# simplify23/MRN

Hardware: NVIDIA B200
Metric: MRN-SVTR 6-expert train samples/s (higher is better)
Workload: dtype bf16

## Files before the change

mrn_b200/csrc/mixer_tc.cu:

```cuda
#include "mixer_tc.h"
#include "sm100.cuh"
#include <stdlib.h>
#include <type_traits>

namespace {

#ifndef MRNB_MIXER_OVL
#define MRNB_MIXER_OVL 1
#endif
constexpr int HD = 32;
constexpr int EPI_WARPS = 8, NTHREADS = 512;
constexpr int REGS_CTRL = 80, REGS_SOFTMAX = 168, REGS_EPI = 96;
constexpr uint32_t Y_COL = 0, S0_COL = 256, S1_COL = 320, O0_COL = 384, O1_COL = 416, STG0_COL = 256, STG1_COL = 352;
constexpr uint32_t STGX_COL = 448;

__device__ __forceinline__ void pair_sync(int q) {
  switch (q) {
    case 0: asm volatile("bar.sync 1, 64;" ::: "memory"); break;
    case 1: asm volatile("bar.sync 2, 64;" ::: "memory"); break;
    case 2: asm volatile("bar.sync 3, 64;" ::: "memory"); break;
    default: asm volatile("bar.sync 4, 64;" ::: "memory"); break;
  }
}
template <int D>
struct MCfg {
  static constexpr int N = 32768 / D;
  static constexpr int NT = N / 128;
  static constexpr int KR = N / 64;
  static constexpr int HEADS = D / HD;
  static constexpr int KB = D / 64;
  static constexpr int A_BYTES = ((D == 128 && MRNB_MIXER_OVL) ? 128 : N) * D * 2;
  static constexpr int HT_BYTES = 128 * HD * 2;
  static constexpr bool OVL = D == 128 && MRNB_MIXER_OVL;
  static constexpr int QKV1_BYTES = 3 * NT * HT_BYTES;
  static constexpr int QKV_BYTES = (OVL ? 2 : 1) * QKV1_BYTES;
  static constexpr int P_TILE = 128 * 64 * 2;
  static constexpr int P_BYTES = 2 * P_TILE;
  static constexpr int WQ_KB_BYTES = 96 * 128;
  static constexpr int WQ_BYTES = KB * WQ_KB_BYTES;
  static constexpr int WP_BYTES = D * HD * 2;
  static constexpr int STG_BYTES = 4 * 2048;
  static constexpr int BIAS_BYTES = OVL ? 4 * 3 * D * 4 : 0;
  static constexpr int SMEM = 1024 + A_BYTES + QKV_BYTES + P_BYTES + WQ_BYTES + 2 * WP_BYTES + STG_BYTES + BIAS_BYTES;
  static_assert(NT * D == 256, "Y accumulator spans 256 TMEM columns");
  static_assert(SMEM <= 227 * 1024, "shared memory budget");
};

struct MixParams {
  const float* bqkv; const float* bproj;
  float* x; long x_gs;
  const float* rowscale; long rs_gs;
  __nv_bfloat16* ln_out; const float* ln_gamma; const float* ln_beta; float ln_eps;
  int upg, total;
  int dbg;
  unsigned long long* trace;
};

#define MIX_TRACE(slot_, idx_)                                                                     \
  do {                                                                                             \
    if (ep.trace && blockIdx.x == 0 && (idx_) < 256) {                                             \
      unsigned long long now__;                                                                    \
      asm volatile("mov.u64 %0, %%globaltimer;" : "=l"(now__));                                    \
      ep.trace[(slot_) * 256 + (idx_)] = now__;                                                    \
    }                                                                                              \
  } while (0)

template <int D, bool LNF, int LNU = 2>
__device__ __forceinline__ void y_tile_epilogue(const MixParams& ep, int e, long unit, int qt, int q, int lane, uint32_t y_addr,
                                                float* xt, float rs, float* stg, uint64_t* release) {
  const int rsub = lane >> 2, c4 = lane & 3;
  const float* bpj = ep.bproj + (long)e * D;
  float sum[4] = {0.f, 0.f, 0.f, 0.f}, sq[4] = {0.f, 0.f, 0.f, 0.f};
  float4 xin[4], xnx[4];
  if (!(ep.dbg & 2)) {
#pragma unroll
// ... 139 lines not shown
      }
    }
    __syncwarp();
  }
}

template <int D, bool LOCAL, bool LNF>
__global__ void __launch_bounds__(NTHREADS, 1)
mixer_tc_kernel(const __grid_constant__ CUtensorMap tmA, const __grid_constant__ CUtensorMap tmWq,
                const __grid_constant__ CUtensorMap tmWp, const MixParams ep) {
  using K = MCfg<D>;
  extern __shared__ uint8_t smem_raw[];
  uint8_t* smem = smem_raw + align_smem_1024_offset(smem_raw);
  uint8_t* sA = smem;
  uint8_t* sQ = sA + K::A_BYTES;
  uint8_t* sK = sQ + K::NT * K::HT_BYTES;
  uint8_t* sV = sK + K::NT * K::HT_BYTES;
  uint8_t* sP = sQ + K::QKV_BYTES;
  uint8_t* sWq = sP + K::P_BYTES;
  uint8_t* sWp = sWq + K::WQ_BYTES;
  uint8_t* sStg = sWp + 2 * K::WP_BYTES;
  float* sBias = reinterpret_cast<float*>(sStg + K::STG_BYTES);
  __shared__ __align__(8) uint64_t a_full, a_empty, wq_full, wq_empty, wp_full[2], wp_empty[2], stg_full[2], stg_empty[2], qkv_ready,
      s_full[2], s_empty[2], p_full[2], o_full[2], so_full[2], so_empty[2], y_full, y_empty[4], st1_done, qkvr[2], qkvf[2], yd[2];
  __shared__ uint32_t tmem_base_sh;
  __shared__ float ln_part[2][4][2][32];

  const int warp = threadIdx.x >> 5, lane = threadIdx.x & 31;
  const int total = ep.total, upg = ep.upg;

  if (threadIdx.x == 0) {
    mbar_init(&a_full, 1); mbar_init(&a_empty, 1); mbar_init(&wq_full, 1); mbar_init(&wq_empty, 1);
    for (int b = 0; b < 2; ++b) {
      mbar_init(&wp_full[b], 1); mbar_init(&wp_empty[b], 2);
      mbar_init(&stg_full[b], 1); mbar_init(&stg_empty[b], K::OVL ? 4 : EPI_WARPS);
      mbar_init(&qkvr[b], 128); mbar_init(&qkvf[b], 2); mbar_init(&yd[b], 1);
      mbar_init(&s_full[b], 1); mbar_init(&s_empty[b], 128); mbar_init(&p_full[b], 128); mbar_init(&o_full[b], 1);
      mbar_init(&so_full[b], 128); mbar_init(&so_empty[b], 1);
    }
    mbar_init(&qkv_ready, EPI_WARPS * 32); mbar_init(&y_full, 2); mbar_init(&st1_done, 1);
    for (int b = 0; b < 4; ++b) mbar_init(&y_empty[b], 4);
    fence_mbarrier_init();
    prefetch_tmap(&tmA);
    prefetch_tmap(&tmWq);
    prefetch_tmap(&tmWp);
  }
  if (warp == 1) tmem_alloc(&tmem_base_sh, 512);
  tc_fence_before();
  __syncthreads();
  tc_fence_after();
  const uint32_t tmem_base = tmem_base_sh;

  auto kr_lo = [](int qt) { return LOCAL ? (2 * qt - 3 > 0 ? 2 * qt - 3 : 0) : 0; };
  auto kr_hi = [](int qt) { return LOCAL ? (2 * qt + 5 < K::KR ? 2 * qt + 5 : K::KR) : K::KR; };

  if (warp < 4) asm volatile("setmaxnreg.dec.sync.aligned.u32 %0;" ::"n"(REGS_CTRL));
  if (warp == 0) {
    if (lane == 0) {
      if constexpr (K::OVL) {
        uint32_t hc = 0, tc = 0;
        for (int u = blockIdx.x; u < total; u += gridDim.x) {
          const int e = u / upg;
          for (int h = 0; h < K::HEADS; ++h, ++hc) {
            mbar_wait(&wq_empty, (hc & 1u) ^ 1u);
            mbar_expect_tx(&wq_full, K::WQ_BYTES);
            for (int kb = 0; kb < K::KB; ++kb)
              for (int part = 0; part < 3; ++part)
                tma_load_3d(sWq + kb * K::WQ_KB_BYTES + part * 4096, &tmWq, &wq_full, kb * 64, part * D + h * HD, e);
            const int buf = hc & 1u;
            mbar_wait(&wp_empty[buf], ((hc >> 1) & 1u) ^ 1u);
            mbar_expect_tx(&wp_full[buf], K::WP_BYTES);
            tma_load_3d(sWp + buf * K::WP_BYTES, &tmWp, &wp_full[buf], h * HD, 0, e);
            for (int mt = 0; mt < K::NT; ++mt, ++tc) {
              mbar_wait(&a_empty, (tc & 1u) ^ 1u);
              mbar_expect_tx(&a_full, K::A_BYTES);
              for (int kb = 0; kb < K::KB; ++kb) tma_load_3d(sA + kb * 16384, &tmA, &a_full, kb * 64, mt * 128, u);
            }
          }
        }
      } else {
      uint32_t hc = 0;
      int i = 0;
      for (int u = blockIdx.x; u < total; u += gridDim.x, ++i) {
        const int e = u / upg;
        mbar_wait(&a_empty, ((uint32_t)i & 1u) ^ 1u);
        mbar_expect_tx(&a_full, K::A_BYTES);
        for (int mt = 0; mt < K::NT; ++mt)
          for (int kb = 0; kb < K::KB; ++kb) tma_load_3d(sA + (mt * K::KB + kb) * 16384, &tmA, &a_full, kb * 64, mt * 128, u);
        for (int h = 0; h < K::HEADS; ++h, ++hc) {
          mbar_wait(&wq_empty, (hc & 1u) ^ 1u);
          mbar_expect_tx(&wq_full, K::WQ_BYTES);
          for (int kb = 0; kb < K::KB; ++kb)
            for (int part = 0; part < 3; ++part)
              tma_load_3d(sWq + kb * K::WQ_KB_BYTES + part * 4096, &tmWq, &wq_full, kb * 64, part * D + h * HD, e);
          const int buf = hc & 1u;
          mbar_wait(&wp_empty[buf], ((hc >> 1) & 1u) ^ 1u);
          mbar_expect_tx(&wp_full[buf], K::WP_BYTES);
          tma_load_3d(sWp + buf * K::WP_BYTES, &tmWp, &wp_full[buf], h * HD, 0, e);
        }
      }
      }
    }
  } else if (warp == 3) {
    if constexpr (K::OVL) {
      if (lane == 0) {
        constexpr uint32_t idesc_qk = umma_idesc(UMMA_BF16, 128, 64), idesc_v = umma_idesc(UMMA_BF16, 128, 32);
        uint32_t hc = 0, tc = 0, pc = 0;
        for (int u = blockIdx.x; u < total; u += gridDim.x) {
          for (int h = 0; h < K::HEADS; ++h, ++hc) {
            mbar_wait(&wq_full, hc & 1u);
            tc_fence_after();
            for (int mt = 0; mt < K::NT; ++mt, ++tc) {
              mbar_wait(&a_full, tc & 1u);
              tc_fence_after();
#pragma unroll
              for (int part = 0; part < 2; ++part, ++pc) {
                mbar_wait(&stg_empty[0], (pc & 1u) ^ 1u);
                tc_fence_after();
                for (int kb = 0; kb < K::KB; ++kb) {
                  const uint64_t ad = umma_desc_k128(smem_u32(sA + kb * 16384));
                  const uint64_t bd = umma_desc_k128(smem_u32(sWq + kb * K::WQ_KB_BYTES + part * 8192));
#pragma unroll
                  for (int k = 0; k < 4; ++k)
                    umma_bf16(tmem_base + STGX_COL, ad + (uint64_t)(k * 2), bd + (uint64_t)(k * 2), part ? idesc_v : idesc_qk, (kb | k) != 0);
                }
                umma_commit(&stg_full[0]);
              }
              umma_commit(&a_empty);
            }
            umma_commit(&wq_empty);
          }
        }
      }
    }
  } else if (warp == 1 || warp == 2) {
    if (lane == 0) {
      const int s = warp == 1 ? 0 : 1;
      constexpr uint32_t idesc_qkv = umma_idesc(UMMA_BF16, 128, 96), idesc_s = umma_idesc(UMMA_BF16, 128, 64);
      constexpr uint32_t idesc_o = umma_idesc(UMMA_BF16, 128, HD, false, true), idesc_y = umma_idesc(UMMA_BF16, 128, D);
      const uint32_t s_col = s ? S1_COL : S0_COL, o_col = s ? O1_COL : O0_COL;
      uint32_t hc = 0, mc = 0, pc = 0, qc = 0;
      bool s_early = false;
      int i = 0;
      for (int u = blockIdx.x; u < total; u += gridDim.x, ++i) {
        if (!K::OVL && s == 0) { mbar_wait(&a_full, (uint32_t)i & 1u); tc_fence_after(); }
        for (int h = 0; h < K::HEADS; ++h, ++hc) {
          if (!K::OVL && s == 0) {
            mbar_wait(&wq_full, hc & 1u);
            mbar_wait(&st1_done, (hc & 1u) ^ 1u);
            tc_fence_after();
            for (int mt = 0; mt < K::NT; ++mt, ++mc) {
              const uint32_t sb = mc & 1u, stg_col = sb ? STG1_COL : STG0_COL;
              mbar_wait(&stg_empty[sb], ((mc >> 1) & 1u) ^ 1u);
              tc_fence_after();
              for (int kb = 0; kb < K::KB; ++kb) {
                const uint64_t ad = umma_desc_k128(smem_u32(sA + (mt * K::KB + kb) * 16384));
                const uint64_t bd = umma_desc_k128(smem_u32(sWq + kb * K::WQ_KB_BYTES));
#pragma unroll
                for (int k = 0; k < 4; ++k) umma_bf16(tmem_base + stg_col, ad + (uint64_t)(k * 2), bd + (uint64_t)(k * 2), idesc_qkv, (kb | k) != 0);
              }
              umma_commit(&stg_full[sb]);
            }
            umma_commit(&wq_empty);
            if (h == K::HEADS - 1) umma_commit(&a_empty);
          }
          const int buf = hc & 1u;
          if constexpr (K::OVL) { if (!s_early) mbar_wait(&qkvr[buf], (hc >> 1) & 1u); }
          else mbar_wait(&qkv_ready, hc & 1u);
// ... 42 lines not shown
                const bool more = !(h == K::HEADS - 1 && u + (int)gridDim.x >= total);
                const uint32_t nb = (hc + 1u) & 1u;
                if (!has_next && more && mbar_test(&qkvr[nb], ((hc + 1u) >> 1) & 1u)) {
                  mbar_wait(&s_empty[s], (pc - 1u) & 1u);
                  tc_fence_after();
                  issue_s_from(sQ + nb * K::QKV1_BYTES, sK + nb * K::QKV1_BYTES, s, kr_lo(s));
                  s_early = true;
                }
              }
              if (last_of_tile) {
                mbar_wait(&so_full[s], qc & 1u);
                tc_fence_after();
                if (!K::OVL && h == 0) { mbar_wait(&y_empty[qt], ((uint32_t)i & 1u) ^ 1u); tc_fence_after(); }
                const uint64_t od = umma_smem_desc(smem_u32(sP + s * K::P_TILE), 16, 512, UMMA_SWIZZLE_64B);
                const uint64_t wd = umma_smem_desc(smem_u32(sWp + buf * K::WP_BYTES), 16, 512, UMMA_SWIZZLE_64B);
#pragma unroll
                for (int k = 0; k < HD / 16; ++k)
                  umma_bf16(tmem_base + Y_COL + (uint32_t)(qt * D), od + (uint64_t)(k * 2), wd + (uint64_t)(k * 2), idesc_y, (h | k) != 0);
                umma_commit(&so_empty[s]);
                if (K::OVL && h == K::HEADS - 1) umma_commit(&yd[s]);
                ++qc;
              }
              if (!has_next) break;
              qt = nqt; kr = nkr;
            }
          }
          umma_commit(&wp_empty[buf]);
          if (s == 1) umma_commit(&st1_done);
          if constexpr (K::OVL) umma_commit(&qkvf[buf]);
        }
        if (!K::OVL) umma_commit(&y_full);
      }
    }
  } else if (warp >= 4 && warp < 12) {
    asm volatile("setmaxnreg.inc.sync.aligned.u32 %0;" ::"n"(REGS_SOFTMAX));
    const int ew = warp - 4, q = warp & 3, ch = ew >> 2;
    const int r = q * 32 + lane;
    const uint32_t lane_addr = tmem_base + ((uint32_t)(q * 32) << 16);
    const int sw = (r >> 1) & 3;
    const float sl2 = 0.17677669529663688110f * 1.4426950408889634f;
    uint8_t* ptile = sP + ch * K::P_TILE;
    float* stg = reinterpret_cast<float*>(ptile + (size_t)q * 4096);
    const int p8 = lane & 7, rsel = lane >> 3;
    constexpr int OW = D / 2, NPASS = OW / 32;
    const uint32_t s_col = ch ? S1_COL : S0_COL, o_col = ch ? O1_COL : O0_COL;
    uint32_t hc = 0, mc = 0, pc = 0, qc = 0;
    int i = 0;
    for (int u = blockIdx.x; u < total; u += gridDim.x, ++i) {
      const int e = u / upg, b = u % upg;
      if constexpr (K::OVL) {
        const char* xl2 = reinterpret_cast<const char*>(ep.x + (long)e * ep.x_gs + (long)b * K::N * D + (long)(ch * 128) * D);
#pragma unroll
        for (int k = 0; k < D / 32; ++k) asm volatile("prefetch.global.L2 [%0];" ::"l"(xl2 + (long)(k * 128 + q * 32 + lane) * 128));
      }
      for (int h = 0; h < K::HEADS; ++h, ++hc) {
        if constexpr (!K::OVL) {
        float bias[3][16];
#pragma unroll
        for (int pi = 0; pi < 3; ++pi) {
          const int p = ch * 3 + pi;
          const float4* bp = reinterpret_cast<const float4*>(ep.bqkv + (long)e * 3 * D + (p >> 1) * D + h * HD + (p & 1) * 16);
#pragma unroll
          for (int j = 0; j < 4; ++j) {
            const float4 t = __ldg(bp + j);
            bias[pi][4 * j] = t.x; bias[pi][4 * j + 1] = t.y; bias[pi][4 * j + 2] = t.z; bias[pi][4 * j + 3] = t.w;
          }
        }
// ... 136 lines not shown
          }
          const float inv = 1.0f / l;
          {
            uint8_t* row = ptile + r * 64;
#pragma unroll
            for (int c4 = 0; c4 < 4; ++c4) {
              uint32_t pk[4];
#pragma unroll
              for (int k2 = 0; k2 < 4; ++k2) pk[k2] = pack_bf16(acc[c4 * 8 + 2 * k2] * inv, acc[c4 * 8 + 2 * k2 + 1] * inv);
              *reinterpret_cast<uint4*>(row + ((c4 ^ sw) * 16)) = make_uint4(pk[0], pk[1], pk[2], pk[3]);
            }
          }
          asm volatile("fence.proxy.async.shared::cta;" ::: "memory");
          mbar_arrive(&so_full[ch]);
          if constexpr (K::OVL) {
            if (h == K::HEADS - 1) {
              if (warp == 4 && lane == 0) MIX_TRACE(11, i);
              const float rs = ep.rowscale ? ep.rowscale[(long)e * ep.rs_gs + b] : 1.0f;
              float* xt = ep.x + (long)e * ep.x_gs + (long)b * K::N * D + (long)(qt * 128 + q * 32) * D;
              if (ep.dbg == 0) {
                y_tile_epilogue_regs<D, LNF, 2>(ep, e, u, qt, q, lane, lane_addr + Y_COL + (uint32_t)(qt * D), xt, rs, stg, 0, 2, &yd[ch], (uint32_t)i & 1u, nullptr);
              } else {
                mbar_wait(&yd[ch], (uint32_t)i & 1u);
                tc_fence_after();
                y_tile_epilogue<D, LNF, 8>(ep, e, u, qt, q, lane, lane_addr + Y_COL + (uint32_t)(qt * D), xt, rs, stg, nullptr);
              }
              tc_fence_before();
              if (warp == 4 && lane == 0) MIX_TRACE(13, i);
            }
          }
        }
      }

    }
  } else if (warp >= 12) {
    asm volatile("setmaxnreg.dec.sync.aligned.u32 %0;" ::"n"(REGS_EPI));
    const int q = warp & 3;
    const uint32_t lane_addr = tmem_base + ((uint32_t)(q * 32) << 16);
    float* stg = reinterpret_cast<float*>(sStg + q * 2048);
    const int rsub = lane >> 2, c4 = lane & 3;
    int d_u = blockIdx.x, d_h = 0, d_part = 0, d_e = -1;
    uint32_t d_pc = 0, d_hc = 0;
    float* wbias = sBias + q * 3 * D;
    auto try_drain = [&]() -> bool {
      if constexpr (!K::OVL) return false;
      if (d_u >= total) return false;
      mbar_wait(&stg_full[0], d_pc & 1u);
      const int hb = d_hc & 1u;
      if (d_part == 0) {
        mbar_wait(&qkvf[hb], ((d_hc >> 1) & 1u) ^ 1u);
        const int e = d_u / upg;
        if (e != d_e) {
          __syncwarp();
          for (int k = lane; k < 3 * D; k += 32) wbias[k] = ep.bqkv[(long)e * 3 * D + k];
          __syncwarp();
          d_e = e;
        }
      }
      tc_fence_after();
      const int mt = d_part >> 1, part = d_part & 1;
      const int r = q * 32 + lane, sw = (r >> 1) & 3;
      uint8_t* qkv = sQ + hb * K::QKV1_BYTES;
      const int nt = part ? 1 : 2;
      for (int tt = 0; tt < nt; ++tt) {
        uint32_t v[32];
        tmem_ld32(lane_addr + STGX_COL + (uint32_t)(tt * 32), v);
        if (tt == nt - 1) {
          tc_fence_before();
          __syncwarp();
          if (lane == 0) mbar_arrive(&stg_empty[0]);
        }
        const int t = part ? 2 : tt;
        const float4* bp = reinterpret_cast<const float4*>(wbias + t * D + d_h * HD);
        uint8_t* row = qkv + (size_t)t * K::NT * K::HT_BYTES + mt * K::HT_BYTES + r * 64;
#pragma unroll
        for (int c = 0; c < 4; ++c) {
          const float4 b0 = bp[2 * c], b1 = bp[2 * c + 1];
          *reinterpret_cast<uint4*>(row + ((c ^ sw) * 16)) = make_uint4(
              pack_bf16(__uint_as_float(v[8 * c]) + b0.x, __uint_as_float(v[8 * c + 1]) + b0.y),
              pack_bf16(__uint_as_float(v[8 * c + 2]) + b0.z, __uint_as_float(v[8 * c + 3]) + b0.w),
              pack_bf16(__uint_as_float(v[8 * c + 4]) + b1.x, __uint_as_float(v[8 * c + 5]) + b1.y),
              pack_bf16(__uint_as_float(v[8 * c + 6]) + b1.z, __uint_as_float(v[8 * c + 7]) + b1.w));
        }
      }
      ++d_pc;
      if (++d_part == 2 * K::NT) {
        asm volatile("fence.proxy.async.shared::cta;" ::: "memory");
        mbar_arrive(&qkvr[hb]);
        if (warp == 12 && lane == 0) MIX_TRACE(14, (int)d_hc);
        d_part = 0; ++d_hc;
        if (++d_h == K::HEADS) { d_h = 0; d_u += gridDim.x; }
      }
      return true;
    };
    if constexpr (K::OVL) {
      while (d_u < total) try_drain();
    } else {
    int i = 0;
    for (int u = blockIdx.x; u < total; u += gridDim.x, ++i) {
      const int e = u / upg, b = u % upg;
      const float rs = ep.rowscale ? ep.rowscale[(long)e * ep.rs_gs + b] : 1.0f;
      float* xunit = ep.x + (long)e * ep.x_gs + (long)b * K::N * D;
      {
        const char* xl2 = reinterpret_cast<const char*>(xunit);
#pragma unroll
        for (int k = 0; k < 8; ++k) asm volatile("prefetch.global.L2 [%0];" ::"l"(xl2 + ((long)(k * 128 + (threadIdx.x - 384))) * 128));
      }
      mbar_wait(&y_full, (uint32_t)i & 1u);
      tc_fence_after();
      if (warp == 12 && lane == 0) MIX_TRACE(11, i);
// ... 30 lines not shown
  using K = MCfg<D>;
  const long units = (long)p.groups * p.units_per_group;
  CUtensorMap tmA, tmWq, tmWp;
  MRNB_TRY(map3(&tmA, p.A, D, K::N, units, 64, 128, CU_TENSOR_MAP_SWIZZLE_128B));
  MRNB_TRY(map3(&tmWq, p.Wqkv, D, 3 * D, p.groups, 64, 32, CU_TENSOR_MAP_SWIZZLE_128B));
  MRNB_TRY(map3(&tmWp, p.Wproj, D, D, p.groups, 32, D, CU_TENSOR_MAP_SWIZZLE_64B));
  MixParams ep{};
  ep.bqkv = p.bqkv; ep.bproj = p.bproj; ep.x = p.x; ep.x_gs = p.x_gstride;
  ep.rowscale = p.rowscale; ep.rs_gs = p.rowscale_gstride;
  ep.ln_out = (__nv_bfloat16*)p.ln_out; ep.ln_gamma = p.ln_gamma; ep.ln_beta = p.ln_beta; ep.ln_eps = p.ln_eps;
  ep.upg = p.units_per_group; ep.total = (int)units;
  { const char* e = getenv("MRNB_MIXER_DBG"); ep.dbg = e ? atoi(e) : 0; }
  ep.trace = (unsigned long long*)g_mixer_trace;
  static bool attr = false;
  static int num_sms = 148;
  if (!attr) {
    cudaFuncSetAttribute(mixer_tc_kernel<D, LOCAL, LNF>, cudaFuncAttributeMaxDynamicSharedMemorySize, K::SMEM);
    int dev = 0;
    cudaGetDevice(&dev);
    cudaDeviceGetAttribute(&num_sms, cudaDevAttrMultiProcessorCount, dev);
    attr = true;
  }
  const int grid = units < num_sms ? (int)units : num_sms;
  mixer_tc_kernel<D, LOCAL, LNF><<<grid, NTHREADS, K::SMEM, st>>>(tmA, tmWq, tmWp, ep);
  MRNB_CHECK_LAUNCH("mixer_tc_kernel");
  return MRNB_OK;
}

}

int mrnb_mixer_tc(const MrnbMixer& p, cudaStream_t st) {
  MRNB_CHECK_ARG(p.A && p.Wqkv && p.bqkv && p.Wproj && p.bproj && p.x && p.groups > 0 && p.units_per_group > 0, "mixer_tc: null/empty argument");
  MRNB_CHECK_ARG(p.D == 64 || p.D == 128 || p.D == 256, "mixer_tc: D must be 64, 128 or 256");
  MRNB_CHECK_ARG(!p.ln_out || (p.D <= 128 && p.ln_gamma && p.ln_beta), "mixer_tc: fused LayerNorm needs D <= 128");
  MRNB_CHECK_ARG(!(p.local && p.D == 256), "mixer_tc: the Local mixer exists for the 64- and 128-wide stages only");
  MRNB_CHECK_ARG(p.x_gstride % 4 == 0, "mixer_tc: misaligned residual stream");
  const double units = (double)p.groups * p.units_per_group, N = 32768.0 / p.D;
  MrnbProfScope prof(MRNB_PROF_MIXER, st, units * (8.0 * N * p.D * p.D + 4.0 * N * N * p.D),
                     units * N * p.D * (2.0 + 8.0 + (p.ln_out ? 2.0 : 0.0)));
#define MRNB_MIX(D_, LOC_) return p.ln_out ? launch_mixer<D_, LOC_, true>(p, st) : launch_mixer<D_, LOC_, false>(p, st);
  if (p.D == 64) { if (p.local) { MRNB_MIX(64, true) } MRNB_MIX(64, false) }
  if (p.D == 128) { if (p.local) { MRNB_MIX(128, true) } MRNB_MIX(128, false) }
  return launch_mixer<256, false, false>(p, st);
#undef MRNB_MIX
}

extern "C" void mrnb_mixer_set_trace(void* device_buffer) { g_mixer_trace = device_buffer; }

extern "C" int mrnb_mixer_bf16(const void* A, const void* Wqkv, const float* bqkv, const void* Wproj, const float* bproj,
                               float* x, const float* rowscale, void* ln_out, const float* ln_gamma, const float* ln_beta,
                               float ln_eps, int units, int D, int local, cudaStream_t stream) {
  MrnbMixer p{};
  p.A = A; p.Wqkv = Wqkv; p.bqkv = bqkv; p.Wproj = Wproj; p.bproj = bproj; p.x = x; p.x_gstride = 0;
  p.rowscale = rowscale; p.rowscale_gstride = 0;
  p.ln_out = ln_out; p.ln_gamma = ln_gamma; p.ln_beta = ln_beta; p.ln_eps = ln_eps;
  p.D = D; p.groups = 1; p.units_per_group = units; p.local = local;
  return mrnb_mixer_tc(p, stream);
}
```

mrn_b200/csrc/svtr.cu:

```cuda
#include "common.cuh"
#include "gemm_f32.h"
#include "gemm_tc.h"
#include "mlp_tc.h"
#include "mixer_tc.h"
#include <stdlib.h>
#include "svtr.h"
#include "expert_util.cuh"

int mrnb_attention_tc(const void* qkv, void* out, int groups, int N, int d, int heads, int H, int W, int local, cudaStream_t st);

namespace {

template <typename OT, int D, int RPW = 4>
__global__ void __launch_bounds__(256)
layernorm_kernel(const float* x, long x_gs, OT* y, long y_gs, const float* __restrict__ gamma,
                 const float* __restrict__ beta, long rows, long rows_per_group, float eps,
                 __nv_bfloat16* __restrict__ y2 = nullptr, long y2_gs = 0, const float* __restrict__ gamma2 = nullptr,
                 const float* __restrict__ beta2 = nullptr, float eps2 = 0.f) {
  constexpr int VPT = D / 32;
  const long row0 = ((long)blockIdx.x * (blockDim.x >> 5) + (threadIdx.x >> 5)) * RPW;
  const int lane = threadIdx.x & 31;
  float v[RPW][VPT];
#pragma unroll
  for (int r = 0; r < RPW; ++r) {
// ... 693 lines not shown
        P.p[MRNB_P_BLOCK0 + MRNB_PB_NORM1_W], P.p[MRNB_P_BLOCK0 + MRNB_PB_NORM1_B], 1e-6f);
    MRNB_CHECK_LAUNCH("embed_kernel");
  }
  mrnb_prof_end(MRNB_PROF_CONV, st);

  static const int DIMS[3] = {64, 128, 256}, DEPTH[3] = {3, 6, 3}, HEADS[3] = {2, 4, 8}, GH[3] = {8, 4, 2};
  static const int OUTS[3] = {128, 256, 512};
  {
    static bool set = false;
    if (!set) {
      const int mx = 2 * 512 * KV_LD * 4;
      cudaFuncSetAttribute(attention_kernel<AT, true>, cudaFuncAttributeMaxDynamicSharedMemorySize, mx);
      cudaFuncSetAttribute(attention_kernel<AT, false>, cudaFuncAttributeMaxDynamicSharedMemorySize, mx);
      set = true;
    }
  }

  for (int b0 = 0; b0 < B; b0 += Bc) {
    const int bc = (B - b0 < Bc) ? (B - b0) : Bc;
    float* x = xall + (size_t)b0 * 32768;
    long x_gs = (long)B * 32768;
    int blk = 0;
    for (int sidx = 0; sidx < 3; ++sidx) {
      const int d = DIMS[sidx], N = 32768 / d, heads = HEADS[sidx], H = GH[sidx], Wd = 64;
      const long rows_g = (long)bc * N;
      for (int j = 0; j < DEPTH[sidx]; ++j, ++blk) {
        const int pb = MRNB_P_BLOCK0 + blk * MRNB_PB_COUNT;
        const bool local = blk < 6;
        const bool fuse_ln = sizeof(AT) == 2 && d <= 128 && (rows_g % 128) == 0;
        if (!(fuse_ln && j > 0) && !(j == 0 && ln1_ready))
          MRNB_TRY(launch_layernorm<AT>(x, x_gs, lnout, rows_g * d, P.p[pb + MRNB_PB_NORM1_W], P.p[pb + MRNB_PB_NORM1_B],
                                        rows_g * I, rows_g, d, 1e-6f, st));
        if (j == 0) ln1_ready = false;
        if (sizeof(AT) == 2 && use_fused_mixer(d)) {
          MrnbMixer mx{};
          mx.A = lnout; mx.Wqkv = P.h[pb + MRNB_PB_QKV_W]; mx.bqkv = P.p[pb + MRNB_PB_QKV_B];
          mx.Wproj = P.h[pb + MRNB_PB_PROJ_W]; mx.bproj = P.p[pb + MRNB_PB_PROJ_B];
          mx.x = x; mx.x_gstride = x_gs;
          if (drop_scales) { mx.rowscale = drop_scales + ((size_t)blk * 2 + 0) * B + b0; mx.rowscale_gstride = (long)12 * 2 * B; }
          if (fuse_ln) { mx.ln_out = lnout; mx.ln_gamma = P.p[pb + MRNB_PB_NORM2_W]; mx.ln_beta = P.p[pb + MRNB_PB_NORM2_B]; mx.ln_eps = 1e-6f; }
          mx.D = d; mx.groups = I; mx.units_per_group = bc; mx.local = local ? 1 : 0;
          MRNB_TRY(mrnb_mixer_tc(mx, st));
        } else {
          LinearArgs a{};
          a.A = lnout; a.lda = d; a.a_gstride = rows_g * d;
          a.W32 = P.p[pb + MRNB_PB_QKV_W]; a.W16 = P.h[pb + MRNB_PB_QKV_W]; a.w_gstride = (long)3 * d * d;
          a.bias = P.p[pb + MRNB_PB_QKV_B]; a.bias_gstride = 3 * d;
          a.out = qkv; a.ldo = 3 * d; a.o_gstride = rows_g * 3 * d; a.out_is_f32 = F32;
          a.M = (int)rows_g; a.N = 3 * d; a.K = d; a.groups = I;
          MRNB_TRY(linear<AT>(a, st));
          {
            const size_t smem = (size_t)2 * N * KV_LD * sizeof(float);
            dim3 grid(I * bc, heads);
            double pairs = (double)N * N;
            if (local) {
              double sh = 0, sw = 0;
              for (int h = 0; h < H; ++h) sh += (h + 3 < H ? h + 3 : H - 1) - (h - 3 > 0 ? h - 3 : 0) + 1;
              for (int w2 = 0; w2 < Wd; ++w2) sw += (w2 + 5 < Wd ? w2 + 5 : Wd - 1) - (w2 - 5 > 0 ? w2 - 5 : 0) + 1;
              pairs = sh * sw;
            }
            MrnbProfScope prof(MRNB_PROF_ATTN, st, 4.0 * 32 * pairs * heads * I * bc,
                               (double)I * bc * N * d * 4 * sizeof(AT));
            if constexpr (sizeof(AT) == 2) {
              MRNB_TRY(mrnb_attention_tc(qkv, att, I * bc, N, d, heads, H, Wd, local ? 1 : 0, st));
            } else {
              if (local) attention_kernel<AT, true><<<grid, N, smem, st>>>(qkv, att, N, d, heads, H, Wd);
              else attention_kernel<AT, false><<<grid, N, smem, st>>>(qkv, att, N, d, heads, H, Wd);
              MRNB_CHECK_LAUNCH("attention_kernel");
            }
          }
          LinearArgs pr{};
          pr.A = att; pr.lda = d; pr.a_gstride = rows_g * d;
          pr.W32 = P.p[pb + MRNB_PB_PROJ_W]; pr.W16 = P.h[pb + MRNB_PB_PROJ_W]; pr.w_gstride = (long)d * d;
          pr.bias = P.p[pb + MRNB_PB_PROJ_B]; pr.bias_gstride = d;
          pr.out = x; pr.ldo = d; pr.o_gstride = x_gs; pr.out_is_f32 = 1; pr.res = x;
          if (drop_scales) {
            pr.rowscale = drop_scales + ((size_t)blk * 2 + 0) * B + b0; pr.rows_per_scale = N;
            pr.rowscale_gstride = (long)12 * 2 * B;
          }
          pr.M = (int)rows_g; pr.N = d; pr.K = d; pr.groups = I;
          if (fuse_ln) { pr.ln_out = lnout; pr.ln_gamma = P.p[pb + MRNB_PB_NORM2_W]; pr.ln_beta = P.p[pb + MRNB_PB_NORM2_B]; pr.ln_eps = 1e-6f; }
          MRNB_TRY(linear<AT>(pr, st));
        }
        if (!fuse_ln)
          MRNB_TRY(launch_layernorm<AT>(x, x_gs, lnout, rows_g * d, P.p[pb + MRNB_PB_NORM2_W], P.p[pb + MRNB_PB_NORM2_B],
                                        rows_g * I, rows_g, d, 1e-6f, st));
        if constexpr (sizeof(AT) == 2) {
          MrnbMlp mp{};
          mp.A = lnout; mp.W1 = P.h[pb + MRNB_PB_FC1_W]; mp.W2 = P.h[pb + MRNB_PB_FC2_W];
          mp.b1 = P.p[pb + MRNB_PB_FC1_B]; mp.b2 = P.p[pb + MRNB_PB_FC2_B];
          mp.x = x; mp.x_gstride = x_gs;
          if (drop_scales) {
            mp.rowscale = drop_scales + ((size_t)blk * 2 + 1) * B + b0; mp.rows_per_scale = N;
            mp.rowscale_gstride = (long)12 * 2 * B;
          }
          if (fuse_ln && j + 1 < DEPTH[sidx]) {
            const int pn = pb + MRNB_PB_COUNT;
            mp.ln_out = lnout; mp.ln_gamma = P.p[pn + MRNB_PB_NORM1_W]; mp.ln_beta = P.p[pn + MRNB_PB_NORM1_B]; mp.ln_eps = 1e-6f;
          }
          if (j + 1 == DEPTH[sidx]) mp.cast_out = att;
          mp.M = (int)rows_g; mp.D = d; mp.groups = I;
          MRNB_TRY(mrnb_mlp_tc(mp, st));
        } else {
          LinearArgs f1{};
          f1.A = lnout; f1.lda = d; f1.a_gstride = rows_g * d;
          f1.W32 = P.p[pb + MRNB_PB_FC1_W]; f1.W16 = P.h[pb + MRNB_PB_FC1_W]; f1.w_gstride = (long)4 * d * d;
          f1.bias = P.p[pb + MRNB_PB_FC1_B]; f1.bias_gstride = 4 * d;
          f1.out = big; f1.ldo = 4 * d; f1.o_gstride = rows_g * 4 * d; f1.out_is_f32 = F32; f1.gelu = 1;
          f1.M = (int)rows_g; f1.N = 4 * d; f1.K = d; f1.groups = I;
          MRNB_TRY(linear<AT>(f1, st));
          LinearArgs f2{};
          f2.A = big; f2.lda = 4 * d; f2.a_gstride = rows_g * 4 * d;
          f2.W32 = P.p[pb + MRNB_PB_FC2_W]; f2.W16 = P.h[pb + MRNB_PB_FC2_W]; f2.w_gstride = (long)4 * d * d;
          f2.bias = P.p[pb + MRNB_PB_FC2_B]; f2.bias_gstride = d;
          f2.out = x; f2.ldo = d; f2.o_gstride = x_gs; f2.out_is_f32 = 1; f2.res = x;
          if (drop_scales) {
            f2.rowscale = drop_scales + ((size_t)blk * 2 + 1) * B + b0; f2.rows_per_scale = N;
// ... 158 lines not shown
```

mrn_b200/ops.py:

```python
from __future__ import annotations

import ctypes as C
from typing import Dict, List, Optional, Sequence

import torch

from . import _lib as L

T_FRAMES = 64
T_FRAMES_CRNN = 63
D_FEAT = 256


def _stream():
    return C.c_void_p(torch.cuda.current_stream().cuda_stream)


def _p(t: Optional[torch.Tensor]):
    if t is None:
        return C.c_void_p(0)
    if not t.is_cuda:
        raise RuntimeError("mrn_b200 ops need CUDA tensors (no CPU fallback)")
    return C.c_void_p(t.data_ptr())

# ... 65 lines not shown
                           % (dtype, tuple(shape), device, out.dtype, tuple(out.shape), out.device))
    return out


def linear_bf16(a, w, bias=None, residual=None, gelu=False, out_f32=True, out=None):
    assert a.dtype == torch.bfloat16 and w.dtype == torch.bfloat16 and a.is_contiguous() and w.is_contiguous()
    _chk_f32(bias, residual)
    M, K = a.shape
    N = w.shape[0]
    out = _out(out, (M, N), a.device, torch.float32 if out_f32 else torch.bfloat16)
    L.check(L.load().mrnb_linear_bf16(_p(a), _p(w), _p(bias), _p(residual), _p(out), int(out_f32), M, N, K, int(gelu),
                                      _stream()), "linear_bf16")
    return out


def tc_gemm_general(a, a_mn, b, b_mn, M, N, K, splitk=1):
    assert a.dtype == torch.bfloat16 and b.dtype == torch.bfloat16 and a.is_contiguous() and b.is_contiguous()
    out = torch.zeros(M, N, device=a.device, dtype=torch.float32)
    L.check(L.load().mrnb_tc_gemm_general(_p(a), int(a_mn), _p(b), int(b_mn), _p(out), M, N, K, int(splitk), _stream()),
            "tc_gemm_general")
    return out


def mlp_bf16(a16, w1_16, b1, w2_16, b2, x, rowscale=None, rows_per_scale=1, ln_gamma=None, ln_beta=None, ln_eps=1e-6):
    assert a16.dtype == torch.bfloat16 and w1_16.dtype == torch.bfloat16 and w2_16.dtype == torch.float16
    _chk_f32(b1, b2, x, rowscale, ln_gamma, ln_beta)
    M, D = x.shape
    ln_out = torch.empty(M, D, device=x.device, dtype=torch.bfloat16) if ln_gamma is not None else None
    L.check(L.load().mrnb_mlp_bf16(_p(a16), _p(w1_16), _p(b1), _p(w2_16), _p(b2), _p(x), _p(rowscale), int(rows_per_scale),
                                   _p(ln_out), _p(ln_gamma), _p(ln_beta), float(ln_eps), M, D, _stream()), "mlp_bf16")
    return ln_out


def mixer_bf16(a16, wqkv16, bqkv, wproj16, bproj, x, local, rowscale=None, ln_gamma=None, ln_beta=None, ln_eps=1e-6):
    assert a16.dtype == torch.bfloat16 and wqkv16.dtype == torch.bfloat16 and wproj16.dtype == torch.bfloat16
    _chk_f32(bqkv, bproj, x, rowscale, ln_gamma, ln_beta)
    units, N, D = x.shape
    assert N * D == 32768 and a16.shape == x.shape and a16.is_contiguous()
    ln_out = torch.empty(units, N, D, device=x.device, dtype=torch.bfloat16) if ln_gamma is not None else None
    L.check(L.load().mrnb_mixer_bf16(_p(a16), _p(wqkv16), _p(bqkv), _p(wproj16), _p(bproj), _p(x), _p(rowscale), _p(ln_out),
                                     _p(ln_gamma), _p(ln_beta), float(ln_eps), units, D, int(local), _stream()), "mixer_bf16")
    return ln_out


def layernorm(x, gamma, beta, eps):
    _chk_f32(x, gamma, beta)
    y = torch.empty_like(x)
    rows = x.numel() // x.shape[-1]
    L.check(L.load().mrnb_layernorm_f32(_p(x), _p(y), _p(gamma), _p(beta), rows, x.shape[-1], float(eps), _stream()), "layernorm")
    return y


def svtr_attention(qkv, heads, H, W, local):
    _chk_f32(qkv)
    G, N, d3 = qkv.shape
    out = torch.empty(G, N, d3 // 3, device=qkv.device, dtype=torch.float32)
    L.check(L.load().mrnb_svtr_attention_f32(_p(qkv), _p(out), G, N, d3 // 3, heads, H, W, int(local), _stream()), "attention")
    return out


def svtr_attention_bf16(qkv, heads, H, W, local, out=None):
    assert qkv.dtype == torch.bfloat16 and qkv.is_contiguous()
    G, N, d3 = qkv.shape
    out = _out(out, (G, N, d3 // 3), qkv.device, torch.bfloat16)
    L.check(L.load().mrnb_svtr_attention_bf16(_p(qkv), _p(out), G, N, d3 // 3, heads, H, W, int(local), _stream()),
            "attention_bf16")
    return out


def attn_tc_train_forward(qkv, heads, W, local, P=None, O=None):
    assert qkv.dtype == torch.bfloat16 and qkv.is_contiguous()
    B, N, d3 = qkv.shape
# ... 703 lines not shown
```

Baseline: 22130.

## Add overlapped K-split pipeline to D=256 mixer with fused LayerNorm

```diff
diff --git a/mrn_b200/csrc/mixer_tc.cu b/mrn_b200/csrc/mixer_tc.cu
--- a/mrn_b200/csrc/mixer_tc.cu
+++ b/mrn_b200/csrc/mixer_tc.cu
@@ -31,7 +31,8 @@
   static constexpr int KB = D / 64;
   static constexpr int A_BYTES = ((D == 128 && MRNB_MIXER_OVL) ? 128 : N) * D * 2;
   static constexpr int HT_BYTES = 128 * HD * 2;
-  static constexpr bool OVL = D == 128 && MRNB_MIXER_OVL;
+  static constexpr bool OVL = (D == 128 && MRNB_MIXER_OVL) || D == 256;
+  static constexpr bool KSPLIT = D == 256;
   static constexpr int QKV1_BYTES = 3 * NT * HT_BYTES;
   static constexpr int QKV_BYTES = (OVL ? 2 : 1) * QKV1_BYTES;
   static constexpr int P_TILE = 128 * 64 * 2;
@@ -39,8 +40,8 @@
   static constexpr int WQ_KB_BYTES = 96 * 128;
   static constexpr int WQ_BYTES = KB * WQ_KB_BYTES;
   static constexpr int WP_BYTES = D * HD * 2;
-  static constexpr int STG_BYTES = 4 * 2048;
-  static constexpr int BIAS_BYTES = OVL ? 4 * 3 * D * 4 : 0;
+  static constexpr int STG_BYTES = KSPLIT ? 0 : 4 * 2048;
+  static constexpr int BIAS_BYTES = (OVL && !KSPLIT) ? 4 * 3 * D * 4 : 0;
   static constexpr int SMEM = 1024 + A_BYTES + QKV_BYTES + P_BYTES + WQ_BYTES + 2 * WP_BYTES + STG_BYTES + BIAS_BYTES;
   static_assert(NT * D == 256, "Y accumulator spans 256 TMEM columns");
   static_assert(SMEM <= 227 * 1024, "shared memory budget");
@@ -246,7 +247,7 @@
   if (threadIdx.x == 0) {
     mbar_init(&a_full, 1); mbar_init(&a_empty, 1); mbar_init(&wq_full, 1); mbar_init(&wq_empty, 1);
     for (int b = 0; b < 2; ++b) {
-      mbar_init(&wp_full[b], 1); mbar_init(&wp_empty[b], 2);
+      mbar_init(&wp_full[b], 1); mbar_init(&wp_empty[b], K::KSPLIT ? 1 : 2);
       mbar_init(&stg_full[b], 1); mbar_init(&stg_empty[b], K::OVL ? 4 : EPI_WARPS);
       mbar_init(&qkvr[b], 128); mbar_init(&qkvf[b], 2); mbar_init(&yd[b], 1);
       mbar_init(&s_full[b], 1); mbar_init(&s_empty[b], 128); mbar_init(&p_full[b], 128); mbar_init(&o_full[b], 1);
@@ -276,20 +277,34 @@
         for (int u = blockIdx.x; u < total; u += gridDim.x) {
           const int e = u / upg;
           for (int h = 0; h < K::HEADS; ++h, ++hc) {
+            if constexpr (K::KSPLIT) {
+              uint64_t* const wqv_full = &stg_full[1];
+              uint64_t* const wqv_empty = &st1_done;
+              for (int p = 0; p < 2; ++p) {
+                uint64_t* const full = p ? wqv_full : &wq_full;
+                mbar_wait(p ? wqv_empty : &wq_empty, (hc & 1u) ^ 1u);
+                mbar_expect_tx(full, (2 - p) * K::KB * 4096);
+                for (int kb = 0; kb < K::KB; ++kb)
+                  for (int part = 2 * p; part < 2 + p; ++part)
+                    tma_load_3d(sWq + kb * K::WQ_KB_BYTES + part * 4096, &tmWq, full, kb * 64, part * D + h * HD, e);
+              }
+            } else {
             mbar_wait(&wq_empty, (hc & 1u) ^ 1u);
             mbar_expect_tx(&wq_full, K::WQ_BYTES);
             for (int kb = 0; kb < K::KB; ++kb)
               for (int part = 0; part < 3; ++part)
                 tma_load_3d(sWq + kb * K::WQ_KB_BYTES + part * 4096, &tmWq, &wq_full, kb * 64, part * D + h * HD, e);
+            }
             const int buf = hc & 1u;
             mbar_wait(&wp_empty[buf], ((hc >> 1) & 1u) ^ 1u);
             mbar_expect_tx(&wp_full[buf], K::WP_BYTES);
             tma_load_3d(sWp + buf * K::WP_BYTES, &tmWp, &wp_full[buf], h * HD, 0, e);
-            for (int mt = 0; mt < K::NT; ++mt, ++tc) {
-              mbar_wait(&a_empty, (tc & 1u) ^ 1u);
-              mbar_expect_tx(&a_full, K::A_BYTES);
-              for (int kb = 0; kb < K::KB; ++kb) tma_load_3d(sA + kb * 16384, &tmA, &a_full, kb * 64, mt * 128, u);
-            }
+            if (!K::KSPLIT || h == 0)
+              for (int mt = 0; mt < K::NT; ++mt, ++tc) {
+                mbar_wait(&a_empty, (tc & 1u) ^ 1u);
+                mbar_expect_tx(&a_full, K::A_BYTES);
+                for (int kb = 0; kb < K::KB; ++kb) tma_load_3d(sA + kb * 16384, &tmA, &a_full, kb * 64, mt * 128, u);
+              }
           }
         }
       } else {
@@ -322,15 +337,28 @@
         uint32_t hc = 0, tc = 0, pc = 0;
         for (int u = blockIdx.x; u < total; u += gridDim.x) {
           for (int h = 0; h < K::HEADS; ++h, ++hc) {
-            mbar_wait(&wq_full, hc & 1u);
+            if constexpr (!K::KSPLIT) mbar_wait(&wq_full, hc & 1u);
             tc_fence_after();
-            for (int mt = 0; mt < K::NT; ++mt, ++tc) {
-              mbar_wait(&a_full, tc & 1u);
+            for (int mt = 0; mt < K::NT; ++mt) {
+              const bool a_first = !K::KSPLIT || h == 0, a_last = !K::KSPLIT || h == K::HEADS - 1;
+              if (a_first) mbar_wait(&a_full, tc & 1u);
               tc_fence_after();
 #pragma unroll
               for (int part = 0; part < 2; ++part, ++pc) {
                 mbar_wait(&stg_empty[0], (pc & 1u) ^ 1u);
                 tc_fence_after();
+                if constexpr (K::KSPLIT) {
+                  mbar_wait(part ? &stg_full[1] : &wq_full, hc & 1u);
+                  tc_fence_after();
+#pragma unroll 1
+                  for (int kb = 0; kb < K::KB; ++kb) {
+                    const uint64_t ad = umma_desc_k128(smem_u32(sA + kb * 16384));
+                    const uint64_t bd = umma_desc_k128(smem_u32(sWq + kb * K::WQ_KB_BYTES + part * 8192));
+#pragma unroll
+                    for (int k = 0; k < 4; ++k)
+                      umma_bf16(tmem_base + STGX_COL, ad + (uint64_t)(k * 2), bd + (uint64_t)(k * 2), part ? idesc_v : idesc_qk, (kb | k) != 0);
+                  }
+                } else {
                 for (int kb = 0; kb < K::KB; ++kb) {
                   const uint64_t ad = umma_desc_k128(smem_u32(sA + kb * 16384));
                   const uint64_t bd = umma_desc_k128(smem_u32(sWq + kb * K::WQ_KB_BYTES + part * 8192));
@@ -338,16 +366,83 @@
                   for (int k = 0; k < 4; ++k)
                     umma_bf16(tmem_base + STGX_COL, ad + (uint64_t)(k * 2), bd + (uint64_t)(k * 2), part ? idesc_v : idesc_qk, (kb | k) != 0);
                 }
+                }
                 umma_commit(&stg_full[0]);
-              }
-              umma_commit(&a_empty);
-            }
-            umma_commit(&wq_empty);
+                if constexpr (K::KSPLIT) umma_commit(part ? &st1_done : &wq_empty);
+              }
+              if (a_last) {
+                umma_commit(&a_empty);
+                ++tc;
+              }
+            }
+            if constexpr (!K::KSPLIT) umma_commit(&wq_empty);
           }
         }
       }
     }
   } else if (warp == 1 || warp == 2) {
+    if constexpr (K::KSPLIT) {
+      if (lane == 0) {
+        const int s = warp == 1 ? 0 : 1;
+        constexpr uint32_t idesc_s = umma_idesc(UMMA_BF16, 128, 64), idesc_o = umma_idesc(UMMA_BF16, 128, HD, false, true);
+        constexpr uint32_t idesc_y = umma_idesc(UMMA_BF16, 128, D);
+        const uint32_t s_col = s ? S1_COL : S0_COL, o_col = s ? O1_COL : O0_COL;
+        auto issue_s = [&](uint32_t qkv_buf) {
+          const uint64_t qd = umma_smem_desc(smem_u32(sQ + qkv_buf * K::QKV1_BYTES), 16, 512, UMMA_SWIZZLE_64B);
+          const uint64_t kd = umma_smem_desc(smem_u32(sK + qkv_buf * K::QKV1_BYTES + s * 4096), 16, 512, UMMA_SWIZZLE_64B);
+#pragma unroll
+          for (int k = 0; k < HD / 16; ++k) umma_bf16(tmem_base + s_col, qd + (uint64_t)(k * 2), kd + (uint64_t)(k * 2), idesc_s, k);
+          umma_commit(&s_full[s]);
+        };
+        uint32_t hc = 0;
+        bool s_early = false;
+        for (int u = blockIdx.x; u < total; u += gridDim.x) {
+          for (int h = 0; h < K::HEADS; ++h, ++hc) {
+            const uint32_t buf = hc & 1u;
+            if (!s_early) {
+              mbar_wait(&qkvr[buf], (hc >> 1) & 1u);
+              tc_fence_after();
+              issue_s(buf);
+            }
+            mbar_wait(&p_full[s], hc & 1u);
+            tc_fence_after();
+            {
+              const uint64_t pd = umma_desc_k128(smem_u32(sP + s * K::P_TILE));
+              const uint64_t vd = umma_smem_desc(smem_u32(sV + buf * K::QKV1_BYTES + s * 4096), 16, 512, UMMA_SWIZZLE_64B);
+#pragma unroll
+              for (int k = 0; k < 64 / 16; ++k)
+                umma_bf16(tmem_base + o_col, pd + (uint64_t)(k * 2), vd + (uint64_t)((k * 16 * 64) >> 4), idesc_o, k != 0);
+              umma_commit(&o_full[s]);
+            }
+            const bool more = !(h == K::HEADS - 1 && u + (int)gridDim.x >= total);
+            if (more && mbar_test(&qkvr[buf ^ 1u], ((hc + 1u) >> 1) & 1u)) {
+              tc_fence_after();
+              issue_s(buf ^ 1u);
+              s_early = true;
+            } else {
+              s_early = false;
+            }
+            if (s == 0) {
+              mbar_wait(&so_full[0], hc & 1u);
+              mbar_wait(&so_full[1], hc & 1u);
+              mbar_wait(&wp_full[buf], (hc >> 1) & 1u);
+              tc_fence_after();
+              const uint64_t wd = umma_smem_desc(smem_u32(sWp + buf * K::WP_BYTES), 16, 512, UMMA_SWIZZLE_64B);
+#pragma unroll
+              for (int k = 0; k < HD / 16; ++k) {
+                const uint64_t od = umma_smem_desc(smem_u32(sP + k * K::P_TILE), 16, 512, UMMA_SWIZZLE_64B);
+                umma_bf16(tmem_base + Y_COL, od + (uint64_t)(k * 2), wd + (uint64_t)(k * 2), idesc_y, (h | k) != 0);
+              }
+              umma_commit(&so_empty[0]);
+              umma_commit(&so_empty[1]);
+              umma_commit(&wp_empty[buf]);
+              if (h == K::HEADS - 1) { umma_commit(&yd[0]); umma_commit(&yd[1]); }
+            }
+            umma_commit(&qkvf[buf]);
+          }
+        }
+      }
+    } else {
     if (lane == 0) {
       const int s = warp == 1 ? 0 : 1;
       constexpr uint32_t idesc_qkv = umma_idesc(UMMA_BF16, 128, 96), idesc_s = umma_idesc(UMMA_BF16, 128, 64);
@@ -456,7 +551,97 @@
         if (!K::OVL) umma_commit(&y_full);
       }
     }
+    }
   } else if (warp >= 4 && warp < 12) {
+    if constexpr (K::KSPLIT) {
+      asm volatile("setmaxnreg.inc.sync.aligned.u32 %0;" ::"n"(REGS_SOFTMAX));
+      const int ch = (warp - 4) >> 2, q = warp & 3;
+      const int r = q * 32 + lane;
+      const uint32_t lane_addr = tmem_base + ((uint32_t)(q * 32) << 16);
+      const int sw = (r >> 1) & 3;
+      const float sl2 = 0.17677669529663688110f * 1.4426950408889634f;
+      uint8_t* ptile = sP + ch * K::P_TILE;
+      float2* ml_own = reinterpret_cast<float2*>(ptile + 8192);
+      const float2* ml_oth = reinterpret_cast<const float2*>(sP + (ch ^ 1) * K::P_TILE + 8192);
+      float* stg = reinterpret_cast<float*>(ptile + (size_t)q * 4096);
+      uint32_t hc = 0;
+      int i = 0;
+      for (int u = blockIdx.x; u < total; u += gridDim.x, ++i) {
+        const int e = u / upg, b = u % upg;
+        const char* xl2 = reinterpret_cast<const char*>(ep.x + (long)e * ep.x_gs + (long)b * K::N * D + (long)(q * 32 + ch * 16) * D);
+#pragma unroll
+        for (int k = 0; k < 4; ++k) asm volatile("prefetch.global.L2 [%0];" ::"l"(xl2 + (long)(k * 32 + lane) * 128));
+        for (int h = 0; h < K::HEADS; ++h, ++hc) {
+          const uint32_t par = hc & 1u;
+          mbar_wait(&s_full[ch], par);
+          tc_fence_after();
+          uint32_t sv[64];
+          tmem_ld32(lane_addr + (ch ? S1_COL : S0_COL), *reinterpret_cast<uint32_t(*)[32]>(&sv[0]));
+          tmem_ld32(lane_addr + (ch ? S1_COL : S0_COL) + 32u, *reinterpret_cast<uint32_t(*)[32]>(&sv[32]));
+          tc_fence_before();
+          float b0 = -INFINITY, b1 = -INFINITY, b2 = -INFINITY, b3 = -INFINITY;
+#pragma unroll
+          for (int c = 0; c < 64; c += 8) {
+            b0 = max3(b0, __uint_as_float(sv[c]), __uint_as_float(sv[c + 1]));
+            b1 = max3(b1, __uint_as_float(sv[c + 2]), __uint_as_float(sv[c + 3]));
+            b2 = max3(b2, __uint_as_float(sv[c + 4]), __uint_as_float(sv[c + 5]));
+            b3 = max3(b3, __uint_as_float(sv[c + 6]), __uint_as_float(sv[c + 7]));
+          }
+          const float m = fmaxf(fmaxf(b0, b1), fmaxf(b2, b3)) * sl2;
+          mbar_wait(&so_empty[ch], par ^ 1u);
+          uint8_t* prow = ptile + r * 128;
+          float l = 0.f;
+#pragma unroll
+          for (int pcs = 0; pcs < 8; ++pcs) {
+            uint32_t pk[4];
+#pragma unroll
+            for (int k2 = 0; k2 < 8; k2 += 2) {
+              const int c = pcs * 8 + k2;
+              const float p0 = ex2_approx(fmaf(__uint_as_float(sv[c]), sl2, -m));
+              const float p1 = ex2_approx(fmaf(__uint_as_float(sv[c + 1]), sl2, -m));
+              l += p0 + p1;
+              pk[k2 >> 1] = pack_bf16(p0, p1);
+            }
+            *reinterpret_cast<uint4*>(prow + ((pcs ^ (r & 7)) * 16)) = make_uint4(pk[0], pk[1], pk[2], pk[3]);
+          }
+          asm volatile("fence.proxy.async.shared::cta;" ::: "memory");
+          mbar_arrive(&p_full[ch]);
+          mbar_wait(&o_full[ch], par);
+          ml_own[r] = make_float2(m, l);
+          mbar_wait(&o_full[ch ^ 1], par);
+          tc_fence_after();
+          pair_sync(q);
+          const float2 mo = ml_oth[r];
+          const float mx = fmaxf(m, mo.x), a_own = ex2_approx(m - mx), a_oth = ex2_approx(mo.x - mx);
+          const float inv = 1.0f / fmaf(l, a_own, mo.y * a_oth);
+          const float f0 = (ch ? a_oth : a_own) * inv, f1 = (ch ? a_own : a_oth) * inv;
+          uint32_t o0[16], o1[16];
+          tmem_ld16(lane_addr + O0_COL + (uint32_t)(ch * 16), o0);
+          tmem_ld16(lane_addr + O1_COL + (uint32_t)(ch * 16), o1);
+          tc_fence_before();
+          uint8_t* row = ptile + r * 64;
+#pragma unroll
+          for (int c2 = 0; c2 < 2; ++c2) {
+            uint32_t pk[4];
+#pragma unroll
+            for (int k2 = 0; k2 < 4; ++k2) {
+              const int j = c2 * 8 + 2 * k2;
+              pk[k2] = pack_bf16(fmaf(__uint_as_float(o0[j]), f0, __uint_as_float(o1[j]) * f1),
+                                 fmaf(__uint_as_float(o0[j + 1]), f0, __uint_as_float(o1[j + 1]) * f1));
+            }
+            *reinterpret_cast<uint4*>(row + (((ch * 2 + c2) ^ sw) * 16)) = make_uint4(pk[0], pk[1], pk[2], pk[3]);
+          }
+          asm volatile("fence.proxy.async.shared::cta;" ::: "memory");
+          mbar_arrive(&so_full[ch]);
+          if (h == K::HEADS - 1) {
+            const float rs = ep.rowscale ? ep.rowscale[(long)e * ep.rs_gs + b] : 1.0f;
+            float* xt = ep.x + (long)e * ep.x_gs + (long)b * K::N * D + (long)(q * 32) * D;
+            y_tile_epilogue_regs<D, LNF, 1>(ep, e, u, 0, q, lane, lane_addr + Y_COL, xt, rs, stg, 2 * ch, 2, &yd[ch], (uint32_t)i & 1u, nullptr);
+            tc_fence_before();
+          }
+        }
+      }
+    } else {
     asm volatile("setmaxnreg.inc.sync.aligned.u32 %0;" ::"n"(REGS_SOFTMAX));
     const int ew = warp - 4, q = warp & 3, ch = ew >> 2;
     const int r = q * 32 + lane;
@@ -659,6 +844,7 @@
         }
       }
 
+    }
     }
   } else if (warp >= 12) {
     asm volatile("setmaxnreg.dec.sync.aligned.u32 %0;" ::"n"(REGS_EPI));
@@ -678,9 +864,11 @@
         mbar_wait(&qkvf[hb], ((d_hc >> 1) & 1u) ^ 1u);
         const int e = d_u / upg;
         if (e != d_e) {
-          __syncwarp();
-          for (int k = lane; k < 3 * D; k += 32) wbias[k] = ep.bqkv[(long)e * 3 * D + k];
-          __syncwarp();
+          if constexpr (!K::KSPLIT) {
+            __syncwarp();
+            for (int k = lane; k < 3 * D; k += 32) wbias[k] = ep.bqkv[(long)e * 3 * D + k];
+            __syncwarp();
+          }
           d_e = e;
         }
       }
@@ -698,11 +886,13 @@
           if (lane == 0) mbar_arrive(&stg_empty[0]);
         }
         const int t = part ? 2 : tt;
-        const float4* bp = reinterpret_cast<const float4*>(wbias + t * D + d_h * HD);
+        const float4* bp = reinterpret_cast<const float4*>((!K::KSPLIT ? wbias : ep.bqkv + (long)d_e * 3 * D) + t * D + d_h * HD);
         uint8_t* row = qkv + (size_t)t * K::NT * K::HT_BYTES + mt * K::HT_BYTES + r * 64;
 #pragma unroll
         for (int c = 0; c < 4; ++c) {
-          const float4 b0 = bp[2 * c], b1 = bp[2 * c + 1];
+          float4 b0, b1;
+          if constexpr (!K::KSPLIT) { b0 = bp[2 * c]; b1 = bp[2 * c + 1]; }
+          else { b0 = __ldg(bp + 2 * c); b1 = __ldg(bp + 2 * c + 1); }
           *reinterpret_cast<uint4*>(row + ((c ^ sw) * 16)) = make_uint4(
               pack_bf16(__uint_as_float(v[8 * c]) + b0.x, __uint_as_float(v[8 * c + 1]) + b0.y),
               pack_bf16(__uint_as_float(v[8 * c + 2]) + b0.z, __uint_as_float(v[8 * c + 3]) + b0.w),
@@ -799,7 +989,7 @@
 int mrnb_mixer_tc(const MrnbMixer& p, cudaStream_t st) {
   MRNB_CHECK_ARG(p.A && p.Wqkv && p.bqkv && p.Wproj && p.bproj && p.x && p.groups > 0 && p.units_per_group > 0, "mixer_tc: null/empty argument");
   MRNB_CHECK_ARG(p.D == 64 || p.D == 128 || p.D == 256, "mixer_tc: D must be 64, 128 or 256");
-  MRNB_CHECK_ARG(!p.ln_out || (p.D <= 128 && p.ln_gamma && p.ln_beta), "mixer_tc: fused LayerNorm needs D <= 128");
+  MRNB_CHECK_ARG(!p.ln_out || (p.ln_gamma && p.ln_beta), "mixer_tc: fused LayerNorm needs gamma and beta");
   MRNB_CHECK_ARG(!(p.local && p.D == 256), "mixer_tc: the Local mixer exists for the 64- and 128-wide stages only");
   MRNB_CHECK_ARG(p.x_gstride % 4 == 0, "mixer_tc: misaligned residual stream");
   const double units = (double)p.groups * p.units_per_group, N = 32768.0 / p.D;
@@ -808,7 +998,7 @@
 #define MRNB_MIX(D_, LOC_) return p.ln_out ? launch_mixer<D_, LOC_, true>(p, st) : launch_mixer<D_, LOC_, false>(p, st);
   if (p.D == 64) { if (p.local) { MRNB_MIX(64, true) } MRNB_MIX(64, false) }
   if (p.D == 128) { if (p.local) { MRNB_MIX(128, true) } MRNB_MIX(128, false) }
-  return launch_mixer<256, false, false>(p, st);
+  MRNB_MIX(256, false)
 #undef MRNB_MIX
 }
 
diff --git a/mrn_b200/csrc/svtr.cu b/mrn_b200/csrc/svtr.cu
--- a/mrn_b200/csrc/svtr.cu
+++ b/mrn_b200/csrc/svtr.cu
@@ -749,13 +749,14 @@
           MRNB_TRY(launch_layernorm<AT>(x, x_gs, lnout, rows_g * d, P.p[pb + MRNB_PB_NORM1_W], P.p[pb + MRNB_PB_NORM1_B],
                                         rows_g * I, rows_g, d, 1e-6f, st));
         if (j == 0) ln1_ready = false;
+        const bool mixer_ln = sizeof(AT) == 2 && d == 256 && use_fused_mixer(d);
         if (sizeof(AT) == 2 && use_fused_mixer(d)) {
           MrnbMixer mx{};
           mx.A = lnout; mx.Wqkv = P.h[pb + MRNB_PB_QKV_W]; mx.bqkv = P.p[pb + MRNB_PB_QKV_B];
           mx.Wproj = P.h[pb + MRNB_PB_PROJ_W]; mx.bproj = P.p[pb + MRNB_PB_PROJ_B];
           mx.x = x; mx.x_gstride = x_gs;
           if (drop_scales) { mx.rowscale = drop_scales + ((size_t)blk * 2 + 0) * B + b0; mx.rowscale_gstride = (long)12 * 2 * B; }
-          if (fuse_ln) { mx.ln_out = lnout; mx.ln_gamma = P.p[pb + MRNB_PB_NORM2_W]; mx.ln_beta = P.p[pb + MRNB_PB_NORM2_B]; mx.ln_eps = 1e-6f; }
+          if (fuse_ln || mixer_ln) { mx.ln_out = lnout; mx.ln_gamma = P.p[pb + MRNB_PB_NORM2_W]; mx.ln_beta = P.p[pb + MRNB_PB_NORM2_B]; mx.ln_eps = 1e-6f; }
           mx.D = d; mx.groups = I; mx.units_per_group = bc; mx.local = local ? 1 : 0;
           MRNB_TRY(mrnb_mixer_tc(mx, st));
         } else {
@@ -799,7 +800,7 @@
           if (fuse_ln) { pr.ln_out = lnout; pr.ln_gamma = P.p[pb + MRNB_PB_NORM2_W]; pr.ln_beta = P.p[pb + MRNB_PB_NORM2_B]; pr.ln_eps = 1e-6f; }
           MRNB_TRY(linear<AT>(pr, st));
         }
-        if (!fuse_ln)
+        if (!fuse_ln && !mixer_ln)
           MRNB_TRY(launch_layernorm<AT>(x, x_gs, lnout, rows_g * d, P.p[pb + MRNB_PB_NORM2_W], P.p[pb + MRNB_PB_NORM2_B],
                                         rows_g * I, rows_g, d, 1e-6f, st));
         if constexpr (sizeof(AT) == 2) {
diff --git a/mrn_b200/ops.py b/mrn_b200/ops.py
--- a/mrn_b200/ops.py
+++ b/mrn_b200/ops.py
@@ -121,12 +121,13 @@
     return ln_out
 
 
-def mixer_bf16(a16, wqkv16, bqkv, wproj16, bproj, x, local, rowscale=None, ln_gamma=None, ln_beta=None, ln_eps=1e-6):
+def mixer_bf16(a16, wqkv16, bqkv, wproj16, bproj, x, local, rowscale=None, ln_gamma=None, ln_beta=None, ln_eps=1e-6,
+               ln_out=None):
     assert a16.dtype == torch.bfloat16 and wqkv16.dtype == torch.bfloat16 and wproj16.dtype == torch.bfloat16
     _chk_f32(bqkv, bproj, x, rowscale, ln_gamma, ln_beta)
     units, N, D = x.shape
     assert N * D == 32768 and a16.shape == x.shape and a16.is_contiguous()
-    ln_out = torch.empty(units, N, D, device=x.device, dtype=torch.bfloat16) if ln_gamma is not None else None
+    ln_out = _out(ln_out, (units, N, D), x.device, torch.bfloat16) if ln_gamma is not None else None
     L.check(L.load().mrnb_mixer_bf16(_p(a16), _p(wqkv16), _p(bqkv), _p(wproj16), _p(bproj), _p(x), _p(rowscale), _p(ln_out),
                                      _p(ln_gamma), _p(ln_beta), float(ln_eps), units, D, int(local), _stream()), "mixer_bf16")
     return ln_out
```

Result: no change. 22240 (median of 6 runs) (+0.5%).
